# klausondrag/FOSVOS

Measured on AMD Instinct MI355X. Metric: online fine-tune frames/sec (854x480), higher is better.
Workload: dtype bf16; 1 GPU; OSVOS_VGG train_online one-shot fine-tune: 1x3x480x854 frame per step, fwd + class-balanced BCE + bwd, fused SGD step every 5 steps (BASELINE.json configs[1]); batch=1, avg_grad_every_n=5, activations=bf16 NHWC, fp32 accumulate, fp32 master weights, parallelism=single GPU

## Files before the change

fosvos_amd/csrc/common.hpp:

```cpp
#pragma once
#include <hip/hip_runtime.h>
#include <stdarg.h>
#include <algorithm>
#include <stdint.h>
#include <stdio.h>
#include <stdlib.h>
#include <string.h>

#include "../../include/fosvos_hip.h"

namespace fosvos {

extern thread_local char g_err[512];

inline int fail(int code, const char *fmt, ...) __attribute__((format(printf, 2, 3)));
inline int fail(int code, const char *fmt, ...) {
    va_list ap;
    va_start(ap, fmt);
    vsnprintf(g_err, sizeof(g_err), fmt, ap);
    va_end(ap);
    return code;
}

#define FOSVOS_HIP_CHECK(expr)                                                                         \
// ... 72 lines not shown
    hipEvent_t vgg_ev[kFosvosVggEvents];
    hipEvent_t resnet_ev[kFosvosResnetEvents];
    bool buckets_recorded;
};
constexpr uint32_t kFosvosCtxMagic = 0x58544346u;
namespace fosvos {
inline int ctx_check(const fosvos_ctx *ctx, const char *who) {
    FOSVOS_REQUIRE(ctx != nullptr, FOSVOS_E_ARG, "%s: null context (fosvos_ctx_create)", who);
    FOSVOS_REQUIRE(ctx->magic == kFosvosCtxMagic, FOSVOS_E_ARG, "%s: not a live fosvos_ctx", who);
    return FOSVOS_OK;
}

#ifdef FOSVOS_LAB_BUILD
inline const char *lab_env(const char *name) { return getenv(name); }
#else
inline const char *lab_env(const char *) { return nullptr; }
#endif
inline int lab_env_int(const char *name, int dflt) {
    const char *e = lab_env(name);
    return e ? atoi(e) : dflt;
}

bool conv_pp_applicable(int N, int H, int W, int in_ch, int out_ch);
int conv_pp_workgroups();
int conv_pp_forward(const uint16_t *x, const uint16_t *w_packed, const float *bias, uint16_t *y, uint16_t *y_pool, int N,
                    int H, int W, int Cin_pad, int Cout, int Co_pad, bool relu, hipStream_t st,
                    const uint8_t *mask_bits = nullptr, uint32_t *codes = nullptr);

bool conv3x3_pool_codes_applicable(int N, int H, int W, int Ci, int Co);

inline int64_t cdiv(int64_t a, int64_t b) { return (a + b - 1) / b; }
inline int roundup(int a, int b) { return (a + b - 1) / b * b; }

typedef uint16_t bf16_t;
typedef __attribute__((ext_vector_type(8))) __bf16 bf16x8;
typedef __attribute__((ext_vector_type(4))) float f32x4;
typedef __attribute__((ext_vector_type(4))) short s16x4;
typedef unsigned int u32x4 __attribute__((__vector_size__(16)));

__device__ __forceinline__ uint16_t f2bf(float f) {
    __bf16 b = (__bf16)f;
    return __builtin_bit_cast(uint16_t, b);
}
__device__ __forceinline__ float bf2f(uint16_t v) { return __uint_as_float(((uint32_t)v) << 16); }
__device__ __forceinline__ uint4 repack8(const float (&f)[8]) {
    uint4 v;
    v.x = __builtin_amdgcn_perm(__float_as_uint(f[1]), __float_as_uint(f[0]), 0x07060302u);
    v.y = __builtin_amdgcn_perm(__float_as_uint(f[3]), __float_as_uint(f[2]), 0x07060302u);
    v.z = __builtin_amdgcn_perm(__float_as_uint(f[5]), __float_as_uint(f[4]), 0x07060302u);
    v.w = __builtin_amdgcn_perm(__float_as_uint(f[7]), __float_as_uint(f[6]), 0x07060302u);
    return v;
}
typedef float fosvos_f32x2 __attribute__((ext_vector_type(2)));
typedef __bf16 fosvos_bf16x2 __attribute__((ext_vector_type(2)));
__device__ __forceinline__ uint32_t pack2bf(float lo, float hi) {
    const fosvos_f32x2 v = {lo, hi};
    return __builtin_bit_cast(uint32_t, __builtin_convertvector(v, fosvos_bf16x2));
}
__device__ __forceinline__ float relu_f(float v) { return __int_as_float(max(__float_as_int(v), 0)); }
__device__ __forceinline__ void unpack8(const uint4 &v, float (&f)[8]) {
    f[0] = __uint_as_float(v.x << 16);
    f[1] = __uint_as_float(v.x & 0xffff0000u);
    f[2] = __uint_as_float(v.y << 16);
    f[3] = __uint_as_float(v.y & 0xffff0000u);
    f[4] = __uint_as_float(v.z << 16);
    f[5] = __uint_as_float(v.z & 0xffff0000u);
// ... 107 lines not shown
```

fosvos_amd/csrc/conv_igemm.hip:

```cpp
#include <stdlib.h>

#include "common.hpp"

using namespace fosvos;

namespace {

constexpr unsigned kReluAfterAdd = 0x100u;
constexpr unsigned kSubsample2 = 0x200u;
constexpr unsigned kNoSplitK = 0x400u;

struct ConvArgs {
    const uint16_t *x;
    const uint16_t *w;
    const float *bias;
    const uint16_t *relu_src;
    const uint8_t *relu_bits;
    const uint16_t *addend;
    void *y;
    uint16_t *y_pool;
    const uint16_t *unpool_g;
    int N, H, W, Cin, Cout, Co_pad;
    int tiles_x, tiles_y;
    unsigned flags;
// ... 53 lines not shown
    static constexpr int WPE = (BM >= 256 || BN < 64) ? 2 : FOSVOS_MID_WPE;
    static_assert(WM * WN == 4 || WM * WN == 8, "4 or 8 waves per workgroup");
    static_assert(TW % 16 == 0 && WAVE_M % 16 == 0 && WAVE_N % 16 == 0, "fragment alignment");
    static_assert(BM % WM == 0 && BN % WN == 0, "wave split");
};

template <int MF, int NF>
struct TapPlan {
    static constexpr int rows_b = MF / 2 > 0 ? MF / 2 : 1;
    static constexpr int per_row = (NF + rows_b - 1) / rows_b;
    static constexpr int nb(int i) {
        const int left = NF - i * per_row;
        return left <= 0 ? 0 : (left < per_row ? left : per_row);
    }
};
template <int MF, int NF, int I, bool NEXT, int V>
__device__ __forceinline__ void sched_row() {
    if constexpr (I < MF) {
        __builtin_amdgcn_sched_group_barrier(0x008, NF, 0);
        if constexpr (NEXT) __builtin_amdgcn_sched_group_barrier(0x100, 1 + TapPlan<MF, NF>::nb(I), 0);
        constexpr int rows_v = V < MF ? V : MF;
        constexpr int nv = I < MF - rows_v ? 0 : (I == MF - 1 ? V - (rows_v - 1) : 1);
        if constexpr (nv > 0) __builtin_amdgcn_sched_group_barrier(0x020, nv, 0);
    }
}
template <int MF, int NF, bool NEXT, int V>
__device__ __forceinline__ void sched_tap() {
    static_assert(MF <= 8, "sched_tap rows");
    sched_row<MF, NF, 0, NEXT, V>(); sched_row<MF, NF, 1, NEXT, V>(); sched_row<MF, NF, 2, NEXT, V>();
    sched_row<MF, NF, 3, NEXT, V>(); sched_row<MF, NF, 4, NEXT, V>(); sched_row<MF, NF, 5, NEXT, V>();
    sched_row<MF, NF, 6, NEXT, V>(); sched_row<MF, NF, 7, NEXT, V>();
}

template <class T, bool OUT_F32, bool UNPOOL = false>
__global__ __launch_bounds__(T::NT) __attribute__((amdgpu_waves_per_eu(2, T::WPE))) void k_conv3x3_igemm(const ConvArgs a) {
    extern __shared__ __attribute__((aligned(16))) uint4 smem[];
    uint4 *sA = smem;
    uint4 *sB = smem + T::A_SLOTS;
#ifdef FOSVOS_IGEMM_PRIO
    __builtin_amdgcn_s_setprio(FOSVOS_IGEMM_PRIO);
#endif

    const int tid = threadIdx.x, lane = tid & 63;
    const int wave = __builtin_amdgcn_readfirstlane(tid >> 6);
    const int wm = wave / T::WN, wn = wave % T::WN;
    int t = blockIdx.x;
    int cb = blockIdx.y;
    if (a.swizzle) {
        const int n_wg = gridDim.x, n_cb = a.Cout / T::BN, n_t = a.n_t;
        const int q8 = n_wg >> 3, r8 = n_wg & 7, xcd = t & 7;
        const int swz = (xcd < r8 ? xcd * (q8 + 1) : r8 * (q8 + 1) + (xcd - r8) * q8) + (t >> 3);
        if (a.swizzle == 1) { t = fast_div(swz, n_cb, a.m_ncb); cb = swz - t * n_cb; }
        else { cb = fast_div(swz, n_t, a.m_nt); t = swz - cb * n_t; }
    }
    const int t_row = fast_div(t, a.tiles_x, a.m_tx);
    const int tx_i = t - t_row * a.tiles_x;
    const int n = fast_div(t_row, a.tiles_y, a.m_ty);
    const int ty_i = t_row - n * a.tiles_y;
    const int y0 = ty_i * T::TH, x0 = tx_i * T::TW;
    const int n0 = cb * T::BN;
    const int H = a.H, W = a.W, Cin = a.Cin;
    const int n_chunks = Cin >> 5;
    const uint16_t *xn = a.x + (int64_t)n * H * W * Cin;

    int a_goff[T::A_IT];
    int a_slot[T::A_IT];
#pragma unroll
    for (int it = 0; it < T::A_IT; ++it) {
        const int idx = it * T::NT + tid;
        const int oct = idx >> 5, within = idx & 31;
        const int kg = within >> 3;
        const int P = oct * 8 + (within & 7);
        a_slot[it] = -1;
        a_goff[it] = -1;
        if (P < T::NPIX) {
            const int hy = P / T::HALO_W, hx = P - hy * T::HALO_W;
            const int gy = y0 + hy - 1, gx = x0 + hx - 1;
            a_slot[it] = kg * T::NPIX_PAD + P;
            if (gy >= 0 && gy < H && gx >= 0 && gx < W) a_goff[it] = ((gy * W + gx) * Cin + kg * 8) * 2;
        }
    }

    f32x4 acc[T::MF][T::NF];
#pragma unroll
    for (int i = 0; i < T::MF; ++i)
#pragma unroll
        for (int j = 0; j < T::NF; ++j) acc[i][j] = f32x4{0.f, 0.f, 0.f, 0.f};

    int a_base[T::MF];
#pragma unroll
    for (int i = 0; i < T::MF; ++i) {
        const int pb = wm * T::WAVE_M + i * 16;
        const int ty = pb / T::TW, tx = pb % T::TW;
        a_base[i] = (lane >> 4) * T::NPIX_PAD + ty * T::HALO_W + tx + (lane & 15);
    }
    const int b_base = (lane >> 4) * T::BN + wn * T::WAVE_N + (lane & 15);

    const int c_begin = a.k_splits > 1 ? blockIdx.z * a.chunks_per_split : 0;
    const int c_end = a.k_splits > 1 ? min(c_begin + a.chunks_per_split, n_chunks) : n_chunks;

    static_assert(T::A_IT <= 6 && T::B_IT <= 9, "prefetch register file");
    uint4 pa0, pa1, pa2, pa3, pa4, pa5, pb0, pb1, pb2, pb3, pb4, pb5, pb6, pb7, pb8;
    [[maybe_unused]] uint4 pa6, pa7, pa8;
    pa0 = pa1 = pa2 = pa3 = pa4 = pa5 = pb0 = pb1 = pb2 = pb3 = pb4 = pb5 = pb6 = pb7 = pb8 = make_uint4(0, 0, 0, 0);
    const int x_bytes = H * W * Cin * 2, w_bytes = (n_chunks * 36 * a.Co_pad - n0) * 16;
    auto x_rsrc = __builtin_amdgcn_make_buffer_rsrc(const_cast<uint16_t *>(xn), 0, x_bytes, 0x00020000);
    auto w_rsrc = __builtin_amdgcn_make_buffer_rsrc(const_cast<uint16_t *>(a.w) + (int64_t)n0 * 8, 0, w_bytes,
                                                    0x00020000);
    static_assert(T::NT % T::BN == 0, "weight staging assumes BN divides the workgroup size");
    const int b_voff = ((tid / T::BN) * a.Co_pad + tid % T::BN) * 16;
    const int b_row_bytes = a.Co_pad * 16;
#define FOSVOS_LD_A(i)                                                                                  \
    if constexpr (i < T::A_IT)                                                                          \
        pa##i = __builtin_bit_cast(uint4, __builtin_amdgcn_raw_buffer_load_b128(x_rsrc, a_goff[i], cc_ * 64, 0));
#define FOSVOS_LD_B(i)                                                                                  \
    if constexpr (i < T::B_IT)                                                                          \
        pb##i = __builtin_bit_cast(uint4, __builtin_amdgcn_raw_buffer_load_b128(                        \
            w_rsrc, b_voff, (cc_ * 36 + i * (T::NT / T::BN)) * b_row_bytes, 0));
#define FOSVOS_LOAD_CHUNK(cc_expr)                                                                      \
    {                                                                                                   \
        const int cc_ = (cc_expr);                                                                      \
        FOSVOS_LD_A(0) FOSVOS_LD_A(1) FOSVOS_LD_A(2) FOSVOS_LD_A(3) FOSVOS_LD_A(4) FOSVOS_LD_A(5)       \
        FOSVOS_LD_B(0) FOSVOS_LD_B(1) FOSVOS_LD_B(2) FOSVOS_LD_B(3) FOSVOS_LD_B(4) FOSVOS_LD_B(5)       \
        FOSVOS_LD_B(6) FOSVOS_LD_B(7) FOSVOS_LD_B(8)                                                    \
    }
#define FOSVOS_ST_A(i)                                                                                  \
    if constexpr (i < T::A_IT) {                                                                        \
        if (a_slot[i] >= 0) sA[a_slot[i]] = pa##i;                                                      \
    }
#define FOSVOS_ST_B(i)                                                                                  \
    if constexpr (i < T::B_IT) {                                                                        \
        if (i * T::NT + tid < T::B_SLOTS) sB[i * T::NT + tid] = pb##i;                                  \
    }
#define FOSVOS_STORE_CHUNK()                                                                            \
    {                                                                                                   \
        FOSVOS_ST_A(0) FOSVOS_ST_A(1) FOSVOS_ST_A(2) FOSVOS_ST_A(3) FOSVOS_ST_A(4) FOSVOS_ST_A(5)       \
        FOSVOS_ST_B(0) FOSVOS_ST_B(1) FOSVOS_ST_B(2) FOSVOS_ST_B(3) FOSVOS_ST_B(4) FOSVOS_ST_B(5)       \
        FOSVOS_ST_B(6) FOSVOS_ST_B(7) FOSVOS_ST_B(8)                                                    \
    }

#define FOSVOS_RD_A(tap_, i_) \
    af[i_] = __builtin_bit_cast(bf16x8, sA[a_base[i_] + ((tap_) / 3) * T::HALO_W + (tap_) % 3]);
#define FOSVOS_RD_B(tap_, buf_, j_) \
    bfr[buf_][j_] = __builtin_bit_cast(bf16x8, sB[b_base + (tap_) * 4 * T::BN + (j_) * 16]);
#define FOSVOS_ROW(tap_, i_)                                                                            \
    if constexpr ((i_) < T::MF) {                                                                       \
        _Pragma("unroll") for (int j = 0; j < T::NF; ++j) acc[i_][j] =                                  \
            __builtin_amdgcn_mfma_f32_16x16x32_bf16(bfr[(tap_) & 1][j], af[i_], acc[i_][j], 0, 0, 0);   \
        if constexpr ((tap_) < 8) {                                                                     \
            FOSVOS_RD_A((tap_) + 1, i_)                                                                 \
            _Pragma("unroll") for (int j = 0; j < TP::nb(i_); ++j)                                      \
                FOSVOS_RD_B((tap_) + 1, ((tap_) + 1) & 1, (i_) * TP::per_row + j)                       \
        }                                                                                               \
    }
#define FOSVOS_TAP(tap_)                                                                                \
    {                                                                                                   \
        FOSVOS_ROW(tap_, 0) FOSVOS_ROW(tap_, 1) FOSVOS_ROW(tap_, 2) FOSVOS_ROW(tap_, 3)                 \
        FOSVOS_ROW(tap_, 4) FOSVOS_ROW(tap_, 5) FOSVOS_ROW(tap_, 6) FOSVOS_ROW(tap_, 7)                 \
        {                                                                                               \
            const int cc_ = cc + 1;                                                                     \
            FOSVOS_LD_B(tap_)                                                                           \
            FOSVOS_LD_A(tap_)                                                                           \
        }                                                                                               \
        sched_tap<T::MF, T::NF, ((tap_) < 8), 1 + ((tap_) < T::A_IT ? 1 : 0)>();                        \
    }

    FOSVOS_STAMP_RT(11)
    FOSVOS_STAMP_AT(0)
    if (c_begin < c_end) FOSVOS_LOAD_CHUNK(c_begin)
    FOSVOS_STAMP_AT(1)
    using TP = TapPlan<T::MF, T::NF>;
    static_assert(T::MF <= 8, "row macros cover up to 8 pixel fragments per wave");
    bf16x8 af[T::MF], bfr[2][T::NF];
    for (int cc = c_begin; cc < c_end; ++cc) {
        if (cc > c_begin) __syncthreads();
        if (cc == c_end - 1) { FOSVOS_STAMP_AT(6) }
        FOSVOS_STORE_CHUNK()
        if (cc == c_begin) { FOSVOS_STAMP_AT(2) }
        if (cc == c_end - 1) { FOSVOS_STAMP_AT(7) }
        __syncthreads();
        if (cc == c_begin) { FOSVOS_STAMP_AT(3) }
#pragma unroll
        for (int i = 0; i < T::MF; ++i) FOSVOS_RD_A(0, i)
#pragma unroll
        for (int j = 0; j < T::NF; ++j) FOSVOS_RD_B(0, 0, j)
        __builtin_amdgcn_sched_group_barrier(0x100, T::MF + T::NF, 0);
        if (cc + 1 == c_end) {
            x_rsrc = __builtin_amdgcn_make_buffer_rsrc(const_cast<uint16_t *>(xn), 0, 0, 0x00020000);
            w_rsrc = __builtin_amdgcn_make_buffer_rsrc(const_cast<uint16_t *>(a.w) + (int64_t)n0 * 8, 0, 0, 0x00020000);
        }
        FOSVOS_TAP(0) FOSVOS_TAP(1) FOSVOS_TAP(2) FOSVOS_TAP(3) FOSVOS_TAP(4) FOSVOS_TAP(5) FOSVOS_TAP(6)
        FOSVOS_TAP(7) FOSVOS_TAP(8)
        if (cc == c_begin) { FOSVOS_STAMP_AT(5) }
    }
    FOSVOS_STAMP_AT(8)

    const int q = lane >> 4, cl = lane & 15;
    if (a.k_splits > 1) {
        float *po = a.partial + (int64_t)blockIdx.z * a.N * H * W * a.Cout;
#pragma unroll
        for (int i = 0; i < T::MF; ++i) {
            const int pix = wm * T::WAVE_M + i * 16 + cl;
            const int gy = y0 + pix / T::TW, gx = x0 + pix % T::TW;
            if (gy < H && gx < W) {
                float *row = po + (((int64_t)n * H + gy) * W + gx) * a.Cout + n0 + wn * T::WAVE_N + q * 4;
#pragma unroll
                for (int j = 0; j < T::NF; ++j)
                    *reinterpret_cast<float4 *>(row + j * 16) =
                        make_float4(acc[i][j][0], acc[i][j][1], acc[i][j][2], acc[i][j][3]);
            }
        }
        return;
    }
    if (OUT_F32) {
        float *yo = reinterpret_cast<float *>(a.y);
#pragma unroll
        for (int j = 0; j < T::NF; ++j) {
            const int co = n0 + wn * T::WAVE_N + j * 16 + q * 4;
            float4 b = make_float4(0.f, 0.f, 0.f, 0.f);
            if (a.bias) b = *reinterpret_cast<const float4 *>(a.bias + co);
#pragma unroll
            for (int i = 0; i < T::MF; ++i) {
                const int pix = wm * T::WAVE_M + i * 16 + cl;
                const int gy = y0 + pix / T::TW, gx = x0 + pix % T::TW;
                if (gy < H && gx < W) {
                    float4 v = make_float4(acc[i][j][0] + b.x, acc[i][j][1] + b.y, acc[i][j][2] + b.z,
                                           acc[i][j][3] + b.w);
                    if (a.flags & FOSVOS_CONV_RELU)
                        v = make_float4(relu_f(v.x), relu_f(v.y), relu_f(v.z), relu_f(v.w));
                    *reinterpret_cast<float4 *>(yo + (((int64_t)n * H + gy) * W + gx) * a.Cout + co) = v;
                }
            }
        }
        return;
    }
    constexpr int VEC_PER_PIX = T::BN / 8;
    constexpr int OUT_N = T::BM * VEC_PER_PIX;
    constexpr int OUT_IT = (OUT_N + T::NT - 1) / T::NT;
    constexpr int PIX_STEP = T::NT / VEC_PER_PIX;
    static_assert(T::NT % VEC_PER_PIX == 0 && PIX_STEP % T::TW == 0, "a thread's output vectors must share a column");
    constexpr int ROW_STEP = PIX_STEP / T::TW;
    const int o_cg = tid % VEC_PER_PIX, o_pix = tid / VEC_PER_PIX;
    const int o_ly = o_pix / T::TW, o_gx = x0 + o_pix % T::TW;
    const int img_bytes = H * W * a.Cout * 2;
    uint16_t *yo = reinterpret_cast<uint16_t *>(a.y);
    int voff[OUT_IT];
#pragma unroll
    for (int it = 0; it < OUT_IT; ++it) {
        const int gy = y0 + o_ly + it * ROW_STEP;
        const bool ok = it * T::NT + tid < OUT_N && gy < H && o_gx < W;
        voff[it] = ok ? ((gy * W + o_gx) * a.Cout + n0 + o_cg * 8) * 2 : -1;
    }
    const bool masked = (a.relu_src || a.relu_bits || a.addend) && !(a.flags & kSubsample2);
    uint4 mk[OUT_IT], ad[OUT_IT];
#pragma unroll
    for (int it = 0; it < OUT_IT; ++it) mk[it] = ad[it] = make_uint4(0, 0, 0, 0);
    if constexpr (UNPOOL) {
        const int OH = (H + 1) >> 1, OW = (W + 1) >> 1;
        auto m_rsrc = __builtin_amdgcn_make_buffer_rsrc(const_cast<uint16_t *>(a.relu_src + (int64_t)n * H * W * a.Cout), 0,
                                                        img_bytes, 0x00020000);
        auto g_rsrc = __builtin_amdgcn_make_buffer_rsrc(const_cast<uint16_t *>(a.unpool_g + (int64_t)n * OH * OW * a.Cout), 0,
                                                        OH * OW * a.Cout * 2, 0x00020000);
#pragma unroll
        for (int it = 0; it < OUT_IT; ++it)
            mk[it] = __builtin_bit_cast(uint4, __builtin_amdgcn_raw_buffer_load_b128(m_rsrc, voff[it], 0, 0));
#pragma unroll
        for (int it = 0; it < OUT_IT; ++it) {
            const int gy = y0 + o_ly + it * ROW_STEP;
            const int goff = voff[it] < 0 ? -1 : (((gy >> 1) * OW + (o_gx >> 1)) * a.Cout + n0 + o_cg * 8) * 2;
            ad[it] = __builtin_bit_cast(uint4, __builtin_amdgcn_raw_buffer_load_b128(g_rsrc, goff, 0, 0));
        }
    } else if (masked && a.relu_bits) {
        auto b_rsrc = __builtin_amdgcn_make_buffer_rsrc(const_cast<uint8_t *>(a.relu_bits + (int64_t)n * H * W * (a.Cout >> 3)), 0,
                                                        img_bytes >> 4, 0x00020000);
#pragma unroll
        for (int it = 0; it < OUT_IT; ++it) {
            const unsigned b = __builtin_amdgcn_raw_buffer_load_b8(b_rsrc, voff[it] < 0 ? -1 : voff[it] >> 4, 0, 0);
            mk[it] = make_uint4((b & 1u) | ((b & 2u) << 15), ((b >> 2) & 1u) | ((b & 8u) << 13), ((b >> 4) & 1u) | ((b & 32u) << 11),
                                ((b >> 6) & 1u) | ((b & 128u) << 9));
        }
        if (a.addend) {
            auto ad_rsrc = __builtin_amdgcn_make_buffer_rsrc(const_cast<uint16_t *>(a.addend + (int64_t)n * H * W * a.Cout), 0,
                                                             img_bytes, 0x00020000);
#pragma unroll
            for (int it = 0; it < OUT_IT; ++it)
                ad[it] = __builtin_bit_cast(uint4, __builtin_amdgcn_raw_buffer_load_b128(ad_rsrc, voff[it], 0, 0));
        }
    } else if (masked) {
        auto m_rsrc = __builtin_amdgcn_make_buffer_rsrc(
            const_cast<uint16_t *>(a.relu_src ? a.relu_src + (int64_t)n * H * W * a.Cout : yo), 0,
            a.relu_src ? img_bytes : 0, 0x00020000);
        auto ad_rsrc = __builtin_amdgcn_make_buffer_rsrc(
            const_cast<uint16_t *>(a.addend ? a.addend + (int64_t)n * H * W * a.Cout : yo), 0,
            a.addend ? img_bytes : 0, 0x00020000);
#pragma unroll
        for (int it = 0; it < OUT_IT; ++it)
            mk[it] = __builtin_bit_cast(uint4, __builtin_amdgcn_raw_buffer_load_b128(m_rsrc, voff[it], 0, 0));
#pragma unroll
        for (int it = 0; it < OUT_IT; ++it)
            ad[it] = __builtin_bit_cast(uint4, __builtin_amdgcn_raw_buffer_load_b128(ad_rsrc, voff[it], 0, 0));
    }
    float4 bias_r[T::NF];
#pragma unroll
    for (int j = 0; j < T::NF; ++j)
        bias_r[j] = a.bias ? *reinterpret_cast<const float4 *>(a.bias + n0 + wn * T::WAVE_N + j * 16 + q * 4)
                           : make_float4(0.f, 0.f, 0.f, 0.f);
    __syncthreads();
    uint16_t *sO = reinterpret_cast<uint16_t *>(smem);
#pragma unroll
    for (int j = 0; j < T::NF; ++j) {
        const int col = wn * T::WAVE_N + j * 16 + q * 4;
        const float4 b = bias_r[j];
#pragma unroll
        for (int i = 0; i < T::MF; ++i) {
            const int pix = wm * T::WAVE_M + i * 16 + cl;
            float v0 = acc[i][j][0] + b.x, v1 = acc[i][j][1] + b.y, v2 = acc[i][j][2] + b.z, v3 = acc[i][j][3] + b.w;
            if (a.flags & FOSVOS_CONV_RELU) {
                v0 = relu_f(v0); v1 = relu_f(v1); v2 = relu_f(v2); v3 = relu_f(v3);
            }
            *reinterpret_cast<uint2 *>(sO + pix * T::OUT_LD + col) = make_uint2(pack2bf(v0, v1), pack2bf(v2, v3));
        }
    }
    if constexpr (UNPOOL) {
        uint16_t *sX = sO + T::BM * T::OUT_LD;
#pragma unroll
        for (int it = 0; it < OUT_IT; ++it)
            if (it * T::NT + tid < OUT_N)
                *reinterpret_cast<uint4 *>(sX + (o_pix + it * PIX_STEP) * T::OUT_LD + o_cg * 8) = mk[it];
    }
    __syncthreads();
    FOSVOS_STAMP_AT(9)
    const uint16_t *s_vec = sO + o_pix * T::OUT_LD + o_cg * 8;
    auto y_rsrc = __builtin_amdgcn_make_buffer_rsrc(yo + (int64_t)n * H * W * a.Cout, 0, img_bytes, 0x00020000);
    if constexpr (UNPOOL) {
        static_assert((T::TW & (T::TW - 1)) == 0 && T::TH % 2 == 0, "window partners are pix ^ 1 and pix ^ TW");
        const uint16_t *sX = sO + T::BM * T::OUT_LD;
        const fosvos_i16x2 one2 = {1, 1}, zero2 = {0, 0};
        const fosvos_i16x2 late_x = (o_pix & 1) ? zero2 : one2;
#pragma unroll
        for (int it = 0; it < OUT_IT; ++it) {
            const int pix = o_pix + it * PIX_STEP;
            if (it * T::NT + tid >= OUT_N) continue;
            const fosvos_i16x2 late_y = (pix & T::TW) ? zero2 : one2;
            const uint4 cv = keep_where_pos_bf16x8(*reinterpret_cast<const uint4 *>(s_vec + it * PIX_STEP * T::OUT_LD), mk[it]);
            const uint4 x1 = *reinterpret_cast<const uint4 *>(sX + (pix ^ 1) * T::OUT_LD + o_cg * 8);
            const uint4 x2 = *reinterpret_cast<const uint4 *>(sX + (pix ^ T::TW) * T::OUT_LD + o_cg * 8);
            const uint4 x3 = *reinterpret_cast<const uint4 *>(sX + (pix ^ T::TW ^ 1) * T::OUT_LD + o_cg * 8);
            auto win = [&](unsigned own_, unsigned p1, unsigned p2, unsigned p3) {
                const fosvos_i16x2 own = __builtin_bit_cast(fosvos_i16x2, own_);
                const fosvos_i16x2 s = (zero2 - own) & (__builtin_bit_cast(fosvos_i16x2, p1) - own - late_x) &
                                       (__builtin_bit_cast(fosvos_i16x2, p2) - own - late_y) &
                                       (__builtin_bit_cast(fosvos_i16x2, p3) - own - late_y);
                return __builtin_bit_cast(unsigned, s >> 15);
            };
            const uint4 routed = make_uint4(ad[it].x & win(mk[it].x, x1.x, x2.x, x3.x), ad[it].y & win(mk[it].y, x1.y, x2.y, x3.y),
                                            ad[it].z & win(mk[it].z, x1.z, x2.z, x3.z), ad[it].w & win(mk[it].w, x1.w, x2.w, x3.w));
            float f[8], r[8];
            unpack8(cv, f);
            unpack8(routed, r);
#pragma unroll
            for (int e = 0; e < 8; ++e) f[e] += r[e];
            __builtin_amdgcn_raw_buffer_store_b128(__builtin_bit_cast(u32x4, pack8(f)), y_rsrc, voff[it], 0, 0);
        }
    } else if (!(a.flags & kSubsample2)) {
        if (masked) {
#pragma unroll
            for (int it = 0; it < OUT_IT; ++it) {
                uint4 v = *reinterpret_cast<const uint4 *>(s_vec + it * PIX_STEP * T::OUT_LD);
                if (a.relu_src || a.relu_bits) v = keep_where_pos_bf16x8(v, mk[it]);
                if (a.addend || (a.flags & kReluAfterAdd)) {
                    float f[8];
                    unpack8(v, f);
                    if (a.addend) {
                        float av[8];
                        unpack8(ad[it], av);
#pragma unroll
                        for (int e = 0; e < 8; ++e) f[e] += av[e];
                    }
                    if (a.flags & kReluAfterAdd) {
#pragma unroll
                        for (int e = 0; e < 8; ++e) f[e] = relu_f(f[e]);
                    }
                    v = pack8(f);
                }
                __builtin_amdgcn_raw_buffer_store_b128(__builtin_bit_cast(u32x4, v), y_rsrc, voff[it], 0, 0);
            }
        } else {
#pragma unroll
            for (int it = 0; it < OUT_IT; ++it)
                __builtin_amdgcn_raw_buffer_store_b128(
                    __builtin_bit_cast(u32x4, *reinterpret_cast<const uint4 *>(s_vec + it * PIX_STEP * T::OUT_LD)), y_rsrc,
                    voff[it], 0, 0);
// ... 179 lines not shown
            if (blocks(TileMid{}) <= 768 && (one_round ? blocks(TileBig{}) < kMinBlocks * 3 / 4 : nb < kMinBlocks / 2)) big = false;
        }
        if (!big) { p.tile = kMid; nb = blocks(TileMid{}); }
    } else if (out_ch == 32) {
        if (pixels >= 256 * 256) { p.tile = kHalf; nb = blocks(TileHalf{}); }
        else { p.tile = kHalfS; nb = blocks(TileHalfS{}); }
    } else {
        if (pixels >= 256 * 256) { p.tile = kSide; nb = blocks(TileSide{}); }
        else { p.tile = kSideS; nb = blocks(TileSideS{}); }
    }
    if (out_ch % 64 == 0) {
        static const char *force = lab_env("FOSVOS_FORCE_TILE");
        if (force && ((atoi(force) >= 0 && atoi(force) <= 2) || atoi(force) == (int)kHalf)) {
            p.tile = (TileId)atoi(force);
            with_tile(p.tile, [&](auto t) { nb = blocks(t); return 0; });
        }
    }
    int ks = 1;
    if (nb < kMinBlocks * 3 / 4) {
        ks = (int)cdiv(kMinBlocks / 2, nb);
        if (ks < 2) ks = 1;
        if (ks > n_chunks) ks = n_chunks;
        if (ks > 16) ks = 16;
    }
#ifdef FOSVOS_STAMP
    if (const char *e = lab_env("FOSVOS_FORCE_KS")) ks = atoi(e);
#endif
    p.chunks_per_split = (int)cdiv(n_chunks, ks);
    p.k_splits = (int)cdiv(n_chunks, p.chunks_per_split);
    p.workspace_bytes = p.k_splits > 1 ? (size_t)p.k_splits * pixels * out_ch * sizeof(float) : 0;
    return p;
}

template <class T, bool OUT_F32, bool UNPOOL = false>
int launch(const ConvArgs &a0, const ConvPlan &plan, hipStream_t st, int in_ch) {
    constexpr int LDS = UNPOOL && 2 * T::LDS_OUT > T::LDS_MAIN ? 2 * T::LDS_OUT : T::LDS_BYTES;
    ConvArgs a = a0;
    a.tiles_x = (int)cdiv(a.W, T::TW);
    a.tiles_y = (int)cdiv(a.H, T::TH);
    a.k_splits = plan.k_splits;
    a.chunks_per_split = plan.chunks_per_split;
#ifdef FOSVOS_STAMP
    a.stamps = g_stamps;
#endif
    const int64_t tiles = (int64_t)a.tiles_x * a.tiles_y * a.N;
    FOSVOS_REQUIRE(tiles <= 0x7fffffff && a.Cout % T::BN == 0, FOSVOS_E_SHAPE, "conv3x3: tile grid");
    if constexpr (LDS > 64 * 1024) {
        static bool once[64];
        int dev = 0;
        FOSVOS_HIP_CHECK(hipGetDevice(&dev));
        if (dev >= 0 && dev < 64 && !once[dev]) {
            FOSVOS_HIP_CHECK(hipFuncSetAttribute(reinterpret_cast<const void *>(k_conv3x3_igemm<T, OUT_F32, UNPOOL>),
                                                 hipFuncAttributeMaxDynamicSharedMemorySize, LDS));
            once[dev] = true;
        }
    }
    if (g_prof_on) {
        static char name[80];
        snprintf(name, sizeof(name), "k_conv3x3_igemm<Tile<%d, %d, %d, %d, %d>, %s, %s>", T::TH, T::TW, T::BN, T::WM, T::WN,
                 OUT_F32 ? "true" : "false", UNPOOL ? "true" : "false");
        prof_begin(name, st, 2.0 * a.N * a.H * a.W * 9.0 * in_ch * a.Cout);
    }
    {
        static const int swz_env = lab_env_int("FOSVOS_IGEMM_SWIZZLE", -1);
        const int n_cb = a.Cout / T::BN;
        a.swizzle = swz_env >= 0 ? swz_env : (tiles * n_cb >= 64 ? 1 : 0);
        if (tiles * n_cb > 0x7fffffff) a.swizzle = 0;
    }
    {
        const int64_t n_cb = a.Cout / T::BN, n_wg = tiles * n_cb;
        a.n_t = (int)tiles;
        a.m_ncb = recip_mul(n_wg, n_cb);
        a.m_nt = recip_mul(n_wg, tiles);
        a.m_tx = recip_mul(tiles, a.tiles_x);
        a.m_ty = recip_mul(tiles, a.tiles_y);
    }
    const dim3 grid = a.swizzle ? dim3((unsigned)(tiles * (a.Cout / T::BN)), 1u, (unsigned)plan.k_splits)
                                : dim3((unsigned)tiles, (unsigned)(a.Cout / T::BN), (unsigned)plan.k_splits);
    hipLaunchKernelGGL((k_conv3x3_igemm<T, OUT_F32, UNPOOL>), grid, dim3(T::NT), LDS, st, a);
    FOSVOS_LAUNCH_CHECK();
    if (plan.k_splits > 1) {
        const int64_t total8 = (a.flags & kSubsample2) ? (int64_t)a.N * ((a.H + 1) >> 1) * ((a.W + 1) >> 1) * (a.Cout / 8)
                                                       : (int64_t)a.N * a.H * a.W * (a.Cout / 8);
        int64_t g = cdiv(total8, 256);
        if (g > 4096) g = 4096;
        FOSVOS_PROF("k_splitk_epilogue", st, 0.0);
        hipLaunchKernelGGL(k_splitk_epilogue, dim3((unsigned)g), dim3(256), 0, st, a, total8);
        FOSVOS_LAUNCH_CHECK();
    }
    return FOSVOS_OK;
}

int dispatch(ConvArgs a, int in_ch, void *workspace, size_t workspace_bytes, hipStream_t st) {
    const bool f32 = (a.flags & FOSVOS_CONV_OUT_F32) != 0;
    if (a.Cout == 32) {
        FOSVOS_REQUIRE(!f32, FOSVOS_E_ARG, "conv3x3: fp32 output is only built for 16-channel outputs");
    } else if (a.Cout % 64 != 0) {
        FOSVOS_REQUIRE(a.Cout == 16, FOSVOS_E_SHAPE, "conv3x3: output channels must be 16, 32 or a multiple of 64 (got %d)",
                       a.Cout);
        FOSVOS_REQUIRE(a.relu_src == nullptr && a.addend == nullptr, FOSVOS_E_ARG,
                       "conv3x3: 16-channel output has no mask/add epilogue");
    } else {
        FOSVOS_REQUIRE(!f32, FOSVOS_E_ARG, "conv3x3: fp32 output is only built for 16-channel outputs");
    }
    ConvPlan plan = make_plan(a.N, a.H, a.W, in_ch, a.Cout);
    if (a.flags & kNoSplitK) {
        plan.k_splits = 1;
        plan.chunks_per_split = roundup(in_ch, 32) / 32;
        plan.workspace_bytes = 0;
    }
    if (plan.k_splits > 1) {
        FOSVOS_REQUIRE(workspace && workspace_bytes >= plan.workspace_bytes, FOSVOS_E_WORKSPACE,
                       "conv3x3: split-K needs %zu workspace bytes, got %zu", plan.workspace_bytes, workspace_bytes);
        a.partial = reinterpret_cast<float *>(workspace);
    }
    if (a.unpool_g)
        return with_tile(plan.tile, [&](auto t) {
            if constexpr (t.BN == 64 && t.BM >= 128) return launch<decltype(t), false, true>(a, plan, st, in_ch);
            return fail(FOSVOS_E_ARG, "conv3x3: no fused pool backward for this tile");
        });
    return with_tile(plan.tile, [&](auto t) {
        if constexpr (t.BN == 16)
            if (f32) return launch<decltype(t), true>(a, plan, st, in_ch);
        return launch<decltype(t), false>(a, plan, st, in_ch);
    });
}

ConvArgs conv_args(const uint16_t *x, const uint16_t *w_packed, void *y, int N, int H, int W, int in_ch, int out_ch) {
    ConvArgs a{};
    a.x = x; a.w = w_packed; a.y = y;
    a.N = N; a.H = H; a.W = W; a.Cin = roundup(in_ch, 32); a.Cout = out_ch; a.Co_pad = roundup(out_ch, 16);
    return a;
}

bool takes_pp(int N, int H, int W, int in_ch, int out_ch, unsigned flags, bool dgrad = false, const void *addend = nullptr) {
    if ((flags & ~FOSVOS_CONV_RELU) || addend) return false;
    if (dgrad) {
        if (lab_env_int("FOSVOS_PP_DGRAD", 1) == 0 || lab_env_int("FOSVOS_PP", -1) == 0) return false;
    } else {
        static const int mode = lab_env_int("FOSVOS_PP", -1);
        if (mode == 0) return false;
    }
    return conv_pp_applicable(N, H, W, roundup(in_ch, 32), out_ch);
}

int check_common(const void *x, const void *w, const void *y, int N, int H, int W, int in_ch, int out_ch,
                 const char *who) {
    FOSVOS_REQUIRE(x && w && y, FOSVOS_E_ARG, "%s: null pointer", who);
    FOSVOS_REQUIRE(N > 0 && H > 0 && W > 0 && in_ch > 0 && out_ch > 0, FOSVOS_E_SHAPE, "%s: bad shape N=%d H=%d W=%d in=%d out=%d",
                   who, N, H, W, in_ch, out_ch);
    FOSVOS_REQUIRE(out_ch % 16 == 0, FOSVOS_E_SHAPE, "%s: output channels %d not a multiple of 16", who, out_ch);
// ... 176 lines not shown
```

fosvos_amd/csrc/conv_wgrad.hip:

```cpp
#include <stdlib.h>

#include "common.hpp"

using namespace fosvos;

namespace {
constexpr int TH = 8;
constexpr int TPIX = TH * 16;
constexpr int HALO_W = 18;
constexpr int BCI = 64;

struct WgArgs {
    const uint16_t *x;
    const uint16_t *dy;
    float *slabs;
    float *bias_part;
    int N, H, W, Ci, Cy, Cor;
    int tiles_x, tiles_y, n_tiles, tiles_per_split;
    int lab;
    int S, n_ci, n_co, xcd_order;
};

typedef __attribute__((address_space(3))) s16x4 *lds_s16x4_ptr;

namespace v2 {
constexpr int XROW = 24;
constexpr int X_BYTES = (TH + 2) * XROW * 128;
constexpr int X_PIECES = (TH + 2) * XROW / 8;

template <bool SIDE>
struct Cfg2 {
    static constexpr int NW = SIDE ? 4 : 8;
    static constexpr int NT = 64 * NW;
    static constexpr int NU = SIDE ? 1 : 2;
    static constexpr int BCO = SIDE ? 16 : 64;
    static constexpr int YPX = SIDE ? 64 : 128;
    static constexpr int Y_BYTES = TPIX * YPX;
    static constexpr int BUF_BYTES = Y_BYTES + X_BYTES;
    static constexpr int LDS_BYTES = 2 * BUF_BYTES;
    static constexpr int Y_PIECES = Y_BYTES / 1024;
    static constexpr int NXIT = (X_PIECES + NW - 1) / NW;
    static constexpr int N_IT = 2 + NXIT;
    static_assert(Y_PIECES == 2 * NW, "two dy pieces per wave, four tile rows apart");
};

typedef __attribute__((address_space(3))) void lds_void;

__device__ __forceinline__ bf16x8 tr_pair16(const char *p, int second) {
    const s16x4 lo = __builtin_amdgcn_ds_read_tr16_b64_v4i16((lds_s16x4_ptr)(p));
    const s16x4 hi = __builtin_amdgcn_ds_read_tr16_b64_v4i16((lds_s16x4_ptr)(p + second));
    typedef __attribute__((ext_vector_type(8))) short s16x8;
    const s16x8 v = __builtin_shufflevector(lo, hi, 0, 1, 2, 3, 4, 5, 6, 7);
    return __builtin_bit_cast(bf16x8, v);
}

#pragma clang diagnostic push
#pragma clang diagnostic ignored "-Winline-asm"
__device__ __forceinline__ void dma16(const __amdgpu_buffer_rsrc_t rsrc, unsigned lds_dst, unsigned voff, unsigned soff) {
    asm volatile("s_mov_b32 m0, %0\n\ts_nop 0\n\tbuffer_load_dwordx4 %1, %2, %3 offen lds"
                 :: "s"(lds_dst), "v"(voff), "s"(rsrc), "s"(soff) : "memory", "m0");
}
#pragma clang diagnostic pop

template <bool SIDE>
__global__ __launch_bounds__(Cfg2<SIDE>::NT) __attribute__((amdgpu_waves_per_eu(SIDE ? 2 : 3, SIDE ? 4 : 3))) void k_wgrad3x3_v2(const WgArgs a) {
    using C = Cfg2<SIDE>;
    constexpr int NW = C::NW, NU = C::NU, YPX = C::YPX, Y_BYTES = C::Y_BYTES, BUF_BYTES = C::BUF_BYTES, N_IT = C::N_IT;
    extern __shared__ __attribute__((aligned(16))) char smem_w[];
    const int tid = threadIdx.x, lane = tid & 63;
    const int wave = __builtin_amdgcn_readfirstlane(tid >> 6);
    const int wc = SIDE ? 0 : wave >> 2, wi = wave & 3;
    int bid = blockIdx.x;
    if (a.xcd_order) {
        const int n_wg = gridDim.x, q8 = n_wg >> 3, r8 = n_wg & 7, xcd = bid & 7;
        bid = (xcd < r8 ? xcd * (q8 + 1) : r8 * (q8 + 1) + (xcd - r8) * q8) + (bid >> 3);
    }
// ... 466 lines not shown
```

Measured before the change: 1255 frames/s.

## Specialize fused pool-backward conv for single K-chunk and prefetch unpool inputs early

Adds a ONE_CHUNK variant of the fused unpool+conv dgrad kernel, used when the input channel count is 32, which drops the next-chunk prefetch and issues the relu_src and unpooled-gradient loads during the MMA taps instead of after them. It also computes the max-pool routing first and reuses the same LDS region for it, so the kernel no longer needs the larger doubled output LDS allocation. That lets a 64-channel igemm workgroup fit on a CU next to a backbone wgrad workgroup, which a static assert now enforces. The early loads keep more registers live during the main loop, and the routing step gains an extra barrier.

Result: no change. 1252 frames/s (-0.2%).

```diff
diff --git a/fosvos_amd/csrc/common.hpp b/fosvos_amd/csrc/common.hpp
--- a/fosvos_amd/csrc/common.hpp
+++ b/fosvos_amd/csrc/common.hpp
@@ -128,6 +128,9 @@
 inline int64_t cdiv(int64_t a, int64_t b) { return (a + b - 1) / b; }
 inline int roundup(int a, int b) { return (a + b - 1) / b * b; }
 
+constexpr int kCuLdsBytes = 160 * 1024;
+constexpr int kWgradBackboneLdsBytes = 2 * (16384 + 30720);
+
 typedef uint16_t bf16_t;
 typedef __attribute__((ext_vector_type(8))) __bf16 bf16x8;
 typedef __attribute__((ext_vector_type(4))) float f32x4;
diff --git a/fosvos_amd/csrc/conv_igemm.hip b/fosvos_amd/csrc/conv_igemm.hip
--- a/fosvos_amd/csrc/conv_igemm.hip
+++ b/fosvos_amd/csrc/conv_igemm.hip
@@ -109,7 +109,7 @@
     sched_row<MF, NF, 6, NEXT, V>(); sched_row<MF, NF, 7, NEXT, V>();
 }
 
-template <class T, bool OUT_F32, bool UNPOOL = false>
+template <class T, bool OUT_F32, bool UNPOOL = false, bool ONE_CHUNK = false>
 __global__ __launch_bounds__(T::NT) __attribute__((amdgpu_waves_per_eu(2, T::WPE))) void k_conv3x3_igemm(const ConvArgs a) {
     extern __shared__ __attribute__((aligned(16))) uint4 smem[];
     uint4 *sA = smem;
@@ -173,8 +173,9 @@
     }
     const int b_base = (lane >> 4) * T::BN + wn * T::WAVE_N + (lane & 15);
 
-    const int c_begin = a.k_splits > 1 ? blockIdx.z * a.chunks_per_split : 0;
-    const int c_end = a.k_splits > 1 ? min(c_begin + a.chunks_per_split, n_chunks) : n_chunks;
+    static_assert(UNPOOL || !ONE_CHUNK, "the one-chunk form is built for the fused pool backward only");
+    const int c_begin = ONE_CHUNK ? 0 : a.k_splits > 1 ? blockIdx.z * a.chunks_per_split : 0;
+    const int c_end = ONE_CHUNK ? 1 : a.k_splits > 1 ? min(c_begin + a.chunks_per_split, n_chunks) : n_chunks;
 
     static_assert(T::A_IT <= 6 && T::B_IT <= 9, "prefetch register file");
     uint4 pa0, pa1, pa2, pa3, pa4, pa5, pb0, pb1, pb2, pb3, pb4, pb5, pb6, pb7, pb8;
@@ -234,17 +235,69 @@
     {                                                                                                   \
         FOSVOS_ROW(tap_, 0) FOSVOS_ROW(tap_, 1) FOSVOS_ROW(tap_, 2) FOSVOS_ROW(tap_, 3)                 \
         FOSVOS_ROW(tap_, 4) FOSVOS_ROW(tap_, 5) FOSVOS_ROW(tap_, 6) FOSVOS_ROW(tap_, 7)                 \
-        {                                                                                               \
+        if constexpr (!ONE_CHUNK) {                                                                     \
             const int cc_ = cc + 1;                                                                     \
             FOSVOS_LD_B(tap_)                                                                           \
             FOSVOS_LD_A(tap_)                                                                           \
         }                                                                                               \
-        sched_tap<T::MF, T::NF, ((tap_) < 8), 1 + ((tap_) < T::A_IT ? 1 : 0)>();                        \
-    }
+        sched_tap<T::MF, T::NF, ((tap_) < 8), ONE_CHUNK ? 0 : 1 + ((tap_) < T::A_IT ? 1 : 0)>();        \
+    }
+
+    constexpr int VEC_PER_PIX = T::BN / 8;
+    constexpr int OUT_N = T::BM * VEC_PER_PIX;
+    constexpr int OUT_IT = (OUT_N + T::NT - 1) / T::NT;
+    constexpr int PIX_STEP = T::NT / VEC_PER_PIX;
+    static_assert(T::NT % VEC_PER_PIX == 0 && PIX_STEP % T::TW == 0, "a thread's output vectors must share a column");
+    constexpr int ROW_STEP = PIX_STEP / T::TW;
+    constexpr bool EARLY = UNPOOL && ONE_CHUNK;
+    int o_cg, o_pix, o_ly, o_gx, img_bytes;
+    int voff[OUT_IT];
+    uint4 mk[OUT_IT], ad[OUT_IT];
+    auto out_plan = [&]() {
+        o_cg = tid % VEC_PER_PIX; o_pix = tid / VEC_PER_PIX;
+        o_ly = o_pix / T::TW; o_gx = x0 + o_pix % T::TW;
+        img_bytes = H * W * a.Cout * 2;
+#pragma unroll
+        for (int it = 0; it < OUT_IT; ++it) {
+            const int gy = y0 + o_ly + it * ROW_STEP;
+            const bool ok = it * T::NT + tid < OUT_N && gy < H && o_gx < W;
+            voff[it] = ok ? ((gy * W + o_gx) * a.Cout + n0 + o_cg * 8) * 2 : -1;
+        }
+    };
+    auto request_unpool_x = [&]() {
+        auto m_rsrc = __builtin_amdgcn_make_buffer_rsrc(const_cast<uint16_t *>(a.relu_src + (int64_t)n * H * W * a.Cout), 0,
+                                                        img_bytes, 0x00020000);
+#pragma unroll
+        for (int it = 0; it < OUT_IT; ++it)
+            mk[it] = __builtin_bit_cast(uint4, __builtin_amdgcn_raw_buffer_load_b128(m_rsrc, voff[it], 0, 0));
+    };
+    constexpr bool G_PAIRED = UNPOOL && ROW_STEP == 1 && OUT_IT % 2 == 0;
+    int goff[OUT_IT];
+    auto unpool_g_plan = [&]() {
+        const int OW = (W + 1) >> 1;
+#pragma unroll
+        for (int it = 0; it < OUT_IT; it += G_PAIRED ? 2 : 1) {
+            const int gy = y0 + o_ly + it * ROW_STEP;
+            goff[it] = voff[it] < 0 ? -1 : (((gy >> 1) * OW + (o_gx >> 1)) * a.Cout + n0 + o_cg * 8) * 2;
+        }
+    };
+    auto request_unpool_g = [&]() {
+        const int OH = (H + 1) >> 1, OW = (W + 1) >> 1;
+        auto g_rsrc = __builtin_amdgcn_make_buffer_rsrc(const_cast<uint16_t *>(a.unpool_g + (int64_t)n * OH * OW * a.Cout), 0,
+                                                        OH * OW * a.Cout * 2, 0x00020000);
+#pragma unroll
+        for (int it = 0; it < OUT_IT; it += G_PAIRED ? 2 : 1)
+            ad[it] = __builtin_bit_cast(uint4, __builtin_amdgcn_raw_buffer_load_b128(g_rsrc, goff[it], 0, 0));
+    };
 
     FOSVOS_STAMP_RT(11)
     FOSVOS_STAMP_AT(0)
     if (c_begin < c_end) FOSVOS_LOAD_CHUNK(c_begin)
+    if constexpr (EARLY) {
+        out_plan();
+        request_unpool_x();
+        unpool_g_plan();
+    }
     FOSVOS_STAMP_AT(1)
     using TP = TapPlan<T::MF, T::NF>;
     static_assert(T::MF <= 8, "row macros cover up to 8 pixel fragments per wave");
@@ -267,7 +320,12 @@
             w_rsrc = __builtin_amdgcn_make_buffer_rsrc(const_cast<uint16_t *>(a.w) + (int64_t)n0 * 8, 0, 0, 0x00020000);
         }
         FOSVOS_TAP(0) FOSVOS_TAP(1) FOSVOS_TAP(2) FOSVOS_TAP(3) FOSVOS_TAP(4) FOSVOS_TAP(5) FOSVOS_TAP(6)
-        FOSVOS_TAP(7) FOSVOS_TAP(8)
+        FOSVOS_TAP(7)
+        if constexpr (EARLY) {
+            __builtin_amdgcn_sched_barrier(0);
+            request_unpool_g();
+        }
+        FOSVOS_TAP(8)
         if (cc == c_begin) { FOSVOS_STAMP_AT(5) }
     }
     FOSVOS_STAMP_AT(8)
@@ -311,41 +369,18 @@
         }
         return;
     }
-    constexpr int VEC_PER_PIX = T::BN / 8;
-    constexpr int OUT_N = T::BM * VEC_PER_PIX;
-    constexpr int OUT_IT = (OUT_N + T::NT - 1) / T::NT;
-    constexpr int PIX_STEP = T::NT / VEC_PER_PIX;
-    static_assert(T::NT % VEC_PER_PIX == 0 && PIX_STEP % T::TW == 0, "a thread's output vectors must share a column");
-    constexpr int ROW_STEP = PIX_STEP / T::TW;
-    const int o_cg = tid % VEC_PER_PIX, o_pix = tid / VEC_PER_PIX;
-    const int o_ly = o_pix / T::TW, o_gx = x0 + o_pix % T::TW;
-    const int img_bytes = H * W * a.Cout * 2;
     uint16_t *yo = reinterpret_cast<uint16_t *>(a.y);
-    int voff[OUT_IT];
-#pragma unroll
-    for (int it = 0; it < OUT_IT; ++it) {
-        const int gy = y0 + o_ly + it * ROW_STEP;
-        const bool ok = it * T::NT + tid < OUT_N && gy < H && o_gx < W;
-        voff[it] = ok ? ((gy * W + o_gx) * a.Cout + n0 + o_cg * 8) * 2 : -1;
-    }
+    if constexpr (!EARLY) out_plan();
     const bool masked = (a.relu_src || a.relu_bits || a.addend) && !(a.flags & kSubsample2);
-    uint4 mk[OUT_IT], ad[OUT_IT];
-#pragma unroll
-    for (int it = 0; it < OUT_IT; ++it) mk[it] = ad[it] = make_uint4(0, 0, 0, 0);
+    if constexpr (!EARLY) {
+#pragma unroll
+        for (int it = 0; it < OUT_IT; ++it) mk[it] = ad[it] = make_uint4(0, 0, 0, 0);
+    }
     if constexpr (UNPOOL) {
-        const int OH = (H + 1) >> 1, OW = (W + 1) >> 1;
-        auto m_rsrc = __builtin_amdgcn_make_buffer_rsrc(const_cast<uint16_t *>(a.relu_src + (int64_t)n * H * W * a.Cout), 0,
-                                                        img_bytes, 0x00020000);
-        auto g_rsrc = __builtin_amdgcn_make_buffer_rsrc(const_cast<uint16_t *>(a.unpool_g + (int64_t)n * OH * OW * a.Cout), 0,
-                                                        OH * OW * a.Cout * 2, 0x00020000);
-#pragma unroll
-        for (int it = 0; it < OUT_IT; ++it)
-            mk[it] = __builtin_bit_cast(uint4, __builtin_amdgcn_raw_buffer_load_b128(m_rsrc, voff[it], 0, 0));
-#pragma unroll
-        for (int it = 0; it < OUT_IT; ++it) {
-            const int gy = y0 + o_ly + it * ROW_STEP;
-            const int goff = voff[it] < 0 ? -1 : (((gy >> 1) * OW + (o_gx >> 1)) * a.Cout + n0 + o_cg * 8) * 2;
-            ad[it] = __builtin_bit_cast(uint4, __builtin_amdgcn_raw_buffer_load_b128(g_rsrc, goff, 0, 0));
+        if constexpr (!EARLY) {
+            request_unpool_x();
+            unpool_g_plan();
+            request_unpool_g();
         }
     } else if (masked && a.relu_bits) {
         auto b_rsrc = __builtin_amdgcn_make_buffer_rsrc(const_cast<uint8_t *>(a.relu_bits + (int64_t)n * H * W * (a.Cout >> 3)), 0,
@@ -384,42 +419,23 @@
                            : make_float4(0.f, 0.f, 0.f, 0.f);
     __syncthreads();
     uint16_t *sO = reinterpret_cast<uint16_t *>(smem);
-#pragma unroll
-    for (int j = 0; j < T::NF; ++j) {
-        const int col = wn * T::WAVE_N + j * 16 + q * 4;
-        const float4 b = bias_r[j];
-#pragma unroll
-        for (int i = 0; i < T::MF; ++i) {
-            const int pix = wm * T::WAVE_M + i * 16 + cl;
-            float v0 = acc[i][j][0] + b.x, v1 = acc[i][j][1] + b.y, v2 = acc[i][j][2] + b.z, v3 = acc[i][j][3] + b.w;
-            if (a.flags & FOSVOS_CONV_RELU) {
-                v0 = relu_f(v0); v1 = relu_f(v1); v2 = relu_f(v2); v3 = relu_f(v3);
-            }
-            *reinterpret_cast<uint2 *>(sO + pix * T::OUT_LD + col) = make_uint2(pack2bf(v0, v1), pack2bf(v2, v3));
-        }
-    }
     if constexpr (UNPOOL) {
-        uint16_t *sX = sO + T::BM * T::OUT_LD;
+        static_assert((T::TW & (T::TW - 1)) == 0 && T::TH % 2 == 0, "window partners are pix ^ 1 and pix ^ TW");
+        static_assert(T::LDS_OUT <= T::LDS_BYTES, "the relu_src tile fits the workgroup's memory");
+        uint16_t *sX = sO;
 #pragma unroll
         for (int it = 0; it < OUT_IT; ++it)
             if (it * T::NT + tid < OUT_N)
                 *reinterpret_cast<uint4 *>(sX + (o_pix + it * PIX_STEP) * T::OUT_LD + o_cg * 8) = mk[it];
-    }
-    __syncthreads();
-    FOSVOS_STAMP_AT(9)
-    const uint16_t *s_vec = sO + o_pix * T::OUT_LD + o_cg * 8;
-    auto y_rsrc = __builtin_amdgcn_make_buffer_rsrc(yo + (int64_t)n * H * W * a.Cout, 0, img_bytes, 0x00020000);
-    if constexpr (UNPOOL) {
-        static_assert((T::TW & (T::TW - 1)) == 0 && T::TH % 2 == 0, "window partners are pix ^ 1 and pix ^ TW");
-        const uint16_t *sX = sO + T::BM * T::OUT_LD;
+        __syncthreads();
         const fosvos_i16x2 one2 = {1, 1}, zero2 = {0, 0};
         const fosvos_i16x2 late_x = (o_pix & 1) ? zero2 : one2;
+        uint4 g_win = make_uint4(0, 0, 0, 0);
 #pragma unroll
         for (int it = 0; it < OUT_IT; ++it) {
             const int pix = o_pix + it * PIX_STEP;
             if (it * T::NT + tid >= OUT_N) continue;
             const fosvos_i16x2 late_y = (pix & T::TW) ? zero2 : one2;
-            const uint4 cv = keep_where_pos_bf16x8(*reinterpret_cast<const uint4 *>(s_vec + it * PIX_STEP * T::OUT_LD), mk[it]);
             const uint4 x1 = *reinterpret_cast<const uint4 *>(sX + (pix ^ 1) * T::OUT_LD + o_cg * 8);
             const uint4 x2 = *reinterpret_cast<const uint4 *>(sX + (pix ^ T::TW) * T::OUT_LD + o_cg * 8);
             const uint4 x3 = *reinterpret_cast<const uint4 *>(sX + (pix ^ T::TW ^ 1) * T::OUT_LD + o_cg * 8);
@@ -430,11 +446,40 @@
                                        (__builtin_bit_cast(fosvos_i16x2, p3) - own - late_y);
                 return __builtin_bit_cast(unsigned, s >> 15);
             };
-            const uint4 routed = make_uint4(ad[it].x & win(mk[it].x, x1.x, x2.x, x3.x), ad[it].y & win(mk[it].y, x1.y, x2.y, x3.y),
-                                            ad[it].z & win(mk[it].z, x1.z, x2.z, x3.z), ad[it].w & win(mk[it].w, x1.w, x2.w, x3.w));
+            if (!G_PAIRED || !(it & 1)) g_win = ad[it];
+            ad[it] = make_uint4(g_win.x & win(mk[it].x, x1.x, x2.x, x3.x), g_win.y & win(mk[it].y, x1.y, x2.y, x3.y),
+                                g_win.z & win(mk[it].z, x1.z, x2.z, x3.z), g_win.w & win(mk[it].w, x1.w, x2.w, x3.w));
+            asm volatile("" : "+v"(ad[it].x), "+v"(ad[it].y), "+v"(ad[it].z), "+v"(ad[it].w));
+            if (it & 1) __builtin_amdgcn_sched_barrier(0);
+        }
+        __syncthreads();
+    }
+#pragma unroll
+    for (int j = 0; j < T::NF; ++j) {
+        const int col = wn * T::WAVE_N + j * 16 + q * 4;
+        const float4 b = bias_r[j];
+#pragma unroll
+        for (int i = 0; i < T::MF; ++i) {
+            const int pix = wm * T::WAVE_M + i * 16 + cl;
+            float v0 = acc[i][j][0] + b.x, v1 = acc[i][j][1] + b.y, v2 = acc[i][j][2] + b.z, v3 = acc[i][j][3] + b.w;
+            if (a.flags & FOSVOS_CONV_RELU) {
+                v0 = relu_f(v0); v1 = relu_f(v1); v2 = relu_f(v2); v3 = relu_f(v3);
+            }
+            *reinterpret_cast<uint2 *>(sO + pix * T::OUT_LD + col) = make_uint2(pack2bf(v0, v1), pack2bf(v2, v3));
+        }
+    }
+    __syncthreads();
+    FOSVOS_STAMP_AT(9)
+    const uint16_t *s_vec = sO + o_pix * T::OUT_LD + o_cg * 8;
+    auto y_rsrc = __builtin_amdgcn_make_buffer_rsrc(yo + (int64_t)n * H * W * a.Cout, 0, img_bytes, 0x00020000);
+    if constexpr (UNPOOL) {
+#pragma unroll
+        for (int it = 0; it < OUT_IT; ++it) {
+            if (it * T::NT + tid >= OUT_N) continue;
+            const uint4 cv = keep_where_pos_bf16x8(*reinterpret_cast<const uint4 *>(s_vec + it * PIX_STEP * T::OUT_LD), mk[it]);
             float f[8], r[8];
             unpack8(cv, f);
-            unpack8(routed, r);
+            unpack8(ad[it], r);
 #pragma unroll
             for (int e = 0; e < 8; ++e) f[e] += r[e];
             __builtin_amdgcn_raw_buffer_store_b128(__builtin_bit_cast(u32x4, pack8(f)), y_rsrc, voff[it], 0, 0);
@@ -680,9 +725,11 @@
     return p;
 }
 
-template <class T, bool OUT_F32, bool UNPOOL = false>
+template <class T, bool OUT_F32, bool UNPOOL = false, bool ONE_CHUNK = false>
 int launch(const ConvArgs &a0, const ConvPlan &plan, hipStream_t st, int in_ch) {
-    constexpr int LDS = UNPOOL && 2 * T::LDS_OUT > T::LDS_MAIN ? 2 * T::LDS_OUT : T::LDS_BYTES;
+    constexpr int LDS = T::LDS_BYTES;
+    static_assert(T::BN != 64 || LDS + kWgradBackboneLdsBytes <= kCuLdsBytes,
+                  "a 64-channel igemm workgroup must fit on a CU beside a backbone weight-gradient workgroup");
     ConvArgs a = a0;
     a.tiles_x = (int)cdiv(a.W, T::TW);
     a.tiles_y = (int)cdiv(a.H, T::TH);
@@ -698,7 +745,7 @@
         int dev = 0;
         FOSVOS_HIP_CHECK(hipGetDevice(&dev));
         if (dev >= 0 && dev < 64 && !once[dev]) {
-            FOSVOS_HIP_CHECK(hipFuncSetAttribute(reinterpret_cast<const void *>(k_conv3x3_igemm<T, OUT_F32, UNPOOL>),
+            FOSVOS_HIP_CHECK(hipFuncSetAttribute(reinterpret_cast<const void *>(k_conv3x3_igemm<T, OUT_F32, UNPOOL, ONE_CHUNK>),
                                                  hipFuncAttributeMaxDynamicSharedMemorySize, LDS));
             once[dev] = true;
         }
@@ -725,7 +772,7 @@
     }
     const dim3 grid = a.swizzle ? dim3((unsigned)(tiles * (a.Cout / T::BN)), 1u, (unsigned)plan.k_splits)
                                 : dim3((unsigned)tiles, (unsigned)(a.Cout / T::BN), (unsigned)plan.k_splits);
-    hipLaunchKernelGGL((k_conv3x3_igemm<T, OUT_F32, UNPOOL>), grid, dim3(T::NT), LDS, st, a);
+    hipLaunchKernelGGL((k_conv3x3_igemm<T, OUT_F32, UNPOOL, ONE_CHUNK>), grid, dim3(T::NT), LDS, st, a);
     FOSVOS_LAUNCH_CHECK();
     if (plan.k_splits > 1) {
         const int64_t total8 = (a.flags & kSubsample2) ? (int64_t)a.N * ((a.H + 1) >> 1) * ((a.W + 1) >> 1) * (a.Cout / 8)
@@ -764,7 +811,10 @@
     }
     if (a.unpool_g)
         return with_tile(plan.tile, [&](auto t) {
-            if constexpr (t.BN == 64 && t.BM >= 128) return launch<decltype(t), false, true>(a, plan, st, in_ch);
+            if constexpr (t.BN == 64 && t.BM >= 128) {
+                if (a.Cin == 32) return launch<decltype(t), false, true, true>(a, plan, st, in_ch);
+                return launch<decltype(t), false, true>(a, plan, st, in_ch);
+            }
             return fail(FOSVOS_E_ARG, "conv3x3: no fused pool backward for this tile");
         });
     return with_tile(plan.tile, [&](auto t) {
diff --git a/fosvos_amd/csrc/conv_wgrad.hip b/fosvos_amd/csrc/conv_wgrad.hip
--- a/fosvos_amd/csrc/conv_wgrad.hip
+++ b/fosvos_amd/csrc/conv_wgrad.hip
@@ -42,6 +42,7 @@
     static constexpr int NXIT = (X_PIECES + NW - 1) / NW;
     static constexpr int N_IT = 2 + NXIT;
     static_assert(Y_PIECES == 2 * NW, "two dy pieces per wave, four tile rows apart");
+    static_assert(SIDE || LDS_BYTES == kWgradBackboneLdsBytes, "common.hpp: the igemm kernels budget their LDS beside this one");
 };
 
 typedef __attribute__((address_space(3))) void lds_void;
```
